# arghyasur1991/Spark-TTS

Measured on AMD Instinct MI355X. Metric: audio samples/sec (whole node), Spark-TTS-0.5B greedy, higher is better.
Workload: dtype bf16 weights + KV, fp32 activations/accumulate (LLM); vocoder: fp32 operands split into 2 bf16 planes, 3 products on the bf16 matrix pipe, fp32 accumulate

## Files before the change

include/sparkmi_debug.h:

```cpp
#ifndef SPARKMI_DEBUG_H
#define SPARKMI_DEBUG_H

#include "sparkmi.h"

#ifdef __cplusplus
extern "C" {
#endif

int smi_llm_time_kernel(smi_llm* h, int kernel, int layer, int iters, float* ms_avg, void* stream);
int smi_llm_debug_stamps(smi_llm* h, int kernel, int layer, double* out);
int smi_llm_engine(smi_llm* h, int32_t* enabled, int32_t* info, char* why, int n);
int smi_llm_set_engine(smi_llm* h, int on);
int smi_llm_engine_plan(const smi_llm_cfg* cfg, int ncu, int32_t* stats);
int smi_llm_engine_stamps(smi_llm* h, double* out, int cap);
int smi_llm_debug_hidden(smi_llm* h, float* out_host, int n);
int smi_llm_debug_read(smi_llm* h, int what, void* out_host, size_t cap, size_t* got);

int smi_llm_debug_set_kv(smi_llm* h, int layer, int slot, int pos0, int n, const float* k_host, const float* v_host);
int smi_llm_debug_get_kv(smi_llm* h, int layer, int slot, int pos0, int n, float* k_host, float* v_host);
int smi_llm_debug_layer(smi_llm* h, int layer, int M, const int32_t* rows_host, const float* hidden_host, int stage);
enum { SMI_PF_GROUPED = 1, SMI_PF_PGEMM = 2 };
int smi_llm_debug_prefill_layer(smi_llm* h, int layer, int stage, int n_seq, const int32_t* seq_host, const float* hidden_host, int family);
int smi_llm_pf_tiles(const int32_t* rows_host, int M, int32_t* out, int cap, int32_t* n);
int smi_llm_debug_raw_stamps(smi_llm* h, unsigned long long* out, int n);
int smi_llm_debug_sample(smi_llm* h, const float* logits_host, int n_rows, uint64_t seed, int use_bound, int32_t* tokens_out);
int smi_llm_debug_penalize(smi_llm* h, const float* logits_host, int n_rows, const uint16_t* hist_host, const smi_penalty_params* pens,
                           const int32_t* emitted_host, float* logits_out, int32_t* argmax_out);
int smi_llm_debug_logprob(smi_llm* h, const float* logits_host, int n_rows, const float* temperature_host, const int32_t* tokens_host,
                          float* lp_out);
// ... 66 lines not shown
```

spark-tts_amd/csrc/smi_llm.hip:

```cpp
#include "smi_common.h"
#include <stdio.h>
#include <string.h>
#include <atomic>
#include <cmath>
#include <cstddef>
#include <map>
#include <mutex>
#include <vector>

namespace {

constexpr int kMaxRows = SMI_MAX_ROWS;
constexpr int kHeadDim = 64;

struct RowDesc {
  int32_t slot, pos, token, flags;
};

struct SampRec {
  int32_t mode;
  int32_t top_k;
  float inv_temp, top_p;
  unsigned long long seed;
  int32_t has_seed, pad;
// ... 1576 lines not shown
      red[(wave * NTB + nb) * 64 + lane] = make_float4(t[0], t[1], t[2], t[3]);
    }
    __syncthreads();
    if (wave < NTB) {
      const int nb = wave, nt = RT ? (g * NTB + nb < ntl ? p.tlist[1 + g * NTB + nb] : NT) : g * NTB + nb;
      if (nt < NT) {
        float4 s = red[(0 * NTB + nb) * 64 + lane];
#pragma unroll
        for (int wv = 1; wv < NW; ++wv) {
          const float4 t = red[(wv * NTB + nb) * 64 + lane];
          s.x += t.x; s.y += t.y; s.z += t.z; s.w += t.w;
        }
        s.x *= rn; s.y *= rn; s.z *= rn; s.w *= rn;
        const int n = nt * 16 + 4 * (lane >> 4);
        const bool valid = em < M;
        if (RT && valid) lm_mask4(p.ctl, p.rows[m0 + em].slot, n, s);
        if (valid && p.Y) {
          float* y = p.Y + (size_t)(m0 + em) * p.V + n;
          if (n + 0 < p.V) y[0] = s.x;
          if (n + 1 < p.V) y[1] = s.y;
          if (n + 2 < p.V) y[2] = s.z;
          if (n + 3 < p.V) y[3] = s.w;
        }
        float bv = -INFINITY;
        int bi = 0x7fffffff;
        const float sv[4] = {s.x, s.y, s.z, s.w};
#pragma unroll
        for (int r = 0; r < 4; ++r)
          if (n + r < p.V && sv[r] > bv) { bv = sv[r]; bi = n + r; }
#pragma unroll
        for (int o = 16; o <= 32; o <<= 1) {
// ... 10 lines not shown
    }
    __syncthreads();
  }
  if (tid < M) {
    float bv = -INFINITY;
    int bi = 0x7fffffff;
#pragma unroll
    for (int nb = 0; nb < NTB; ++nb) {
      const float ov = bestv[nb * 32 + tid];
      const int oi = besti[nb * 32 + tid];
      if (ov > bv || (ov == bv && oi < bi)) { bv = ov; bi = oi; }
    }
    p.pval[(size_t)(m0 + tid) * gridDim.x + blockIdx.x] = bv;
    p.pidx[(size_t)(m0 + tid) * gridDim.x + blockIdx.x] = bi;
  }
}


template <int UW, int RT = 0>
__global__ __launch_bounds__(256) void k_lm32(GemmP p, int ngroups_arg, int m0) {
  constexpr int NTB = 2, NW = 4, U = UW;
  extern __shared__ __attribute__((aligned(16))) unsigned char smem[];
  const int tid = threadIdx.x, lane = tid & 63, wave = tid >> 6;
  const int KT = p.KT, NT = p.NT;
  const int ntl = RT ? p.tlist[0] : 0;
  const int ngroups = RT ? (ntl + NTB - 1) / NTB : ngroups_arg;
  const int M = p.M - m0 < 32 ? p.M - m0 : 32;
  float4* red = (float4*)smem;
  float* rarr = (float*)(smem + (size_t)NW * NTB * 2 * 1024);
  float* bestv = rarr + 32;
// ... 1644 lines not shown
  float* apart; size_t apart_floats;
  int slot_busy[kMaxRows], slot_len[kMaxRows];
  int slot_plen[kMaxRows];
  uint64_t handle_id, session_gen;
  std::vector<unsigned char> host_blob;
  int do_sample, top_k; float temperature, top_p; unsigned long long seed;
  uint8_t slot_feat[kMaxRows];
  int lm_restrict;
  int seq_dirty[kMaxRows];
  SeqRec* seq;
  std::vector<SeqRec> hseq;
  int32_t* pctx;
  std::vector<int32_t> host_pctx;
  int* tlist;
  std::vector<int32_t> host_tlist;
  float* lp;
  float* lp_part; float2* lp_rowc;
  uint16_t* phist;
  int64_t* poll_dev; int64_t* poll_host;
  int32_t* pen_idx; size_t pen_idx_cap;
  std::vector<int32_t> host_pen_idx;
  float* logits; int* tok;
  float* cand_v; int* cand_i; unsigned int* cand_n;
  unsigned long long* stamps; int stamps_on;
  int max_steps;
  int tune[4];
  int graph_steps;
  int pf_inline;
  int pf_qkv_eighths;
  int prefetch_mask, prefetch_rows;
// ... 546 lines not shown
      break;
  }
  return p;
}

AttnP attn_operands(const smi_llm* L, int layer, const Work& w, const RowDesc* rows, int M) {
  const smi_llm_cfg& c = L->cfg;
  AttnP a;
  memset(&a, 0, sizeof(a));
  a.q = w.q; a.kcache = kv_layer(L, L->kcache, layer); a.vcache = kv_layer(L, L->vcache, layer);
  a.rows = rows; a.xs_out = w.xs_attn; a.M = M; a.q_dim = L->Q; a.n_kv = c.num_kv_heads;
  a.group = c.num_heads / c.num_kv_heads; a.max_pos = c.max_positions; a.n_heads = c.num_heads; a.km = kv_map(L);
  return a;
}

int launch_one(smi_llm* L, int which, int layer, const RowDesc* rows, int M, float* logits, hipStream_t st) {
  const smi_llm_cfg& c = L->cfg;
  const bool fused = fuse_o_now(L, rows, M);
  GemmP p = gemm_operands(L, which, layer, L->dec, rows, M, L->NTh * 4);
  if (which == KLM) p.Y = logits ? logits : (logits_needed(L, step_feat(L)) ? L->logits : nullptr);
  if (L->exact) {
    switch (which) {
      case KQKV: return launch_gemm_x<PRO_NORM, EPI_QKV>(L, p, st);
      case KO: return launch_gemm_x<PRO_PLAIN, EPI_RESID>(L, p, st);
      case KGU: return launch_gemm_x<PRO_NORM, EPI_SWIGLU>(L, p, st);
      case KD: return launch_gemm_x<PRO_PLAIN, EPI_RESID>(L, p, st);
      case KLM:
        SMI_REQUIRE((L->NTlm + 3) / 4 <= L->lm_cap, "lm_head partial buffer too small");
        return launch_gemm_x<PRO_NORM, EPI_LM>(L, p, st);
    }
// ... 55 lines not shown
        return launch_down_chains(L, p, st);
      switch (L->tune[3]) {
        case 2: return launch_gemm<1, 16, 3, 4, PRO_PLAIN, EPI_RESID>(L, p, st);
        case 4: return launch_gemm<1, 8, 10, 2, PRO_PLAIN, EPI_RESID>(L, p, st);
        case 5: return launch_gemm<1, 16, 2, 5, PRO_PLAIN, EPI_RESID, 2>(L, p, st);
        case 6: return launch_gemm<1, 16, 2, 5, PRO_PLAIN, EPI_RESID>(L, p, st);
        default:
          if (M <= 8) return launch_gemm<1, 16, 2, 5, PRO_PLAIN, EPI_RESID, 4>(L, p, st);
          if (M <= 16) return launch_gemm<1, 16, 2, 5, PRO_PLAIN, EPI_RESID, 4, 0>(L, p, st);
          if (M <= 32) return launch_gemm<1, 16, 2, 5, PRO_PLAIN, EPI_RESID, 2, 0>(L, p, st);
          return launch_gemm<1, 16, 2, 5, PRO_PLAIN, EPI_RESID, 1, 0>(L, p, st);
      }
    case KLM: {
      const unsigned feat = step_feat(L);
      p.stamps = L->stamps_on ? L->stamps : nullptr;
      if (L->KTh <= 32 && !logits && rows == L->rows && lm_restricted(L, feat)) {
        p.tlist = L->tlist; p.ctl = L->ctl;
        const size_t lds = (size_t)4 * 2 * 1024 + 32 * 4 + 2 * 32 * 8;
        const size_t lds32 = (size_t)4 * 2 * 2 * 1024 + 32 * 4 + 2 * 32 * 8 + (size_t)L->KTh * 12 * 16 * 16;
        if (M <= 16) {
          hipLaunchKernelGGL((k_lm<1, 1>), dim3(L->lm_blocks), dim3(256), lds, st, p, 0, 0);
          SMI_LAUNCH_CHECK();
          return SMI_OK;
        }
        for (int m0 = 0; m0 < M; m0 += 32) {
          if (!(L->tune2 & 8192) && lds32 <= 150 * 1024) {
            if (L->KTh <= 28) hipLaunchKernelGGL((k_lm32<7, 1>), dim3(lm_blocks_for(L, M)), dim3(256), lds32, st, p, 0, m0);
            else hipLaunchKernelGGL((k_lm32<8, 1>), dim3(lm_blocks_for(L, M)), dim3(256), lds32, st, p, 0, m0);
          } else
            hipLaunchKernelGGL((k_lm<2, 1>), dim3(lm_blocks_for(L, M)), dim3(512), 2 * lds, st, p, 0, m0);
// ... 14 lines not shown
              if (L->KTh <= 28) hipLaunchKernelGGL(k_lm32<7>, dim3(lm_blocks_for(L, M)), dim3(256), lds32, st, p, ngroups, m0);
              else hipLaunchKernelGGL(k_lm32<8>, dim3(lm_blocks_for(L, M)), dim3(256), lds32, st, p, ngroups, m0);
            } else
              hipLaunchKernelGGL(k_lm<2>, dim3(lm_blocks_for(L, M)), dim3(512), 2 * lds, st, p, ngroups, m0);
            SMI_LAUNCH_CHECK();
          }
        }
        return SMI_OK;
      }
      SMI_REQUIRE((L->NTlm + 3) / 4 <= L->lm_cap, "lm_head partial buffer too small");
      return launch_gemm<4, 4, 2, 1, PRO_NORM, EPI_LM>(L, p, st);
    }
    case KFIN: {
      const unsigned feat = step_feat(L);
      FinP f = fin_params(L, M);
      if (feat & F_NGRAM) {
        size_t lds;
        const NgramP np = ngram_params(L, &lds);
        hipLaunchKernelGGL(k_ngram_ban, dim3(1, M), dim3(256), lds, st, np);
        SMI_LAUNCH_CHECK();
      }
      if ((feat & (F_PEN | F_BIAS | F_NGRAM)) || ((feat & F_ALLOW) && logits_needed(L, feat))) {
        PenP pp = pen_params(L, M);
        if (feat & F_BIAS) pp.seq = L->seq;
        hipLaunchKernelGGL(k_penalize, dim3((pp.nblk + kPenWaves - 1) / kPenWaves, M), dim3(256), 0, st, pp);
        SMI_LAUNCH_CHECK();
        f.phist = L->phist;
      }
      if (feat & F_SAMPLE) {
        const SampleP sp = sample_params(L, M);
// ... 407 lines not shown
    for (int i = 0; i < 4; ++i) { const char* e = smi_env(names[i]); L->pg_forced |= e != nullptr; L->pg_min[i] = e ? atoi(e) : common ? L->pgemm_min_rows : dflt[i]; }
  }
  { const char* e = smi_env("SPARKMI_PG_SPLIT_ROWS"); L->pg_split_rows = e ? atoi(e) : kPgSplitRows; if (L->pg_split_rows > kPgSplitRows) L->pg_split_rows = kPgSplitRows; }
  { const char* e = smi_env("SPARKMI_PF_LONG"); L->pf_long = e ? atoi(e) : kMaxRows + 1; if (L->pf_long < kMaxRows + 1) L->pf_long = kMaxRows + 1; }
  { const char* e = smi_env("SPARKMI_GU1_ROWS"); L->gu1_rows = e ? atoi(e) : 32; }
  { const char* e = smi_env("SPARKMI_GU1_LO"); L->gu1_lo = e ? atoi(e) : 4; }
  L->wd_parts = cfg->wd_plain ? 0 : 1;
  L->exact = cfg->weights_exact;
  if (L->exact) L->fuse_o = 0;
  L->pf_tiles = nullptr; L->pf_tiles_cap = 0; L->pf_ntiles = 0;
  L->dbg_pf_rows = 0;
  { const char* e = smi_env("SPARKMI_ATTN_PF2"); L->attn_pf2 = !(e && e[0] == '0'); }
  L->graph = nullptr; L->graph_id = 0; slots_clear(L);
  L->lp = nullptr; L->lp_part = nullptr; L->lp_rowc = nullptr;
  L->tlist = nullptr;
  memset(L->seq_dirty, 0, sizeof(L->seq_dirty));
  L->seq = nullptr; L->hseq.assign(kMaxRows, SeqRec{});
  L->pctx = nullptr;
  L->poll_dev = nullptr; L->poll_host = nullptr;
  L->phist = nullptr; L->pen_idx = nullptr; L->pen_idx_cap = 0; L->plan = nullptr; L->plan_cap = 0; L->B = 0; L->started = 0; L->ctl = nullptr; L->admit_seq = 0; memset(&L->hctl, 0, sizeof(L->hctl));
  L->session = 0; L->identity_slots = 1; L->attn_seg = 1; L->apart = nullptr; L->apart_floats = 0; memset(L->slot_busy, 0, sizeof(L->slot_busy)); memset(L->slot_len, 0, sizeof(L->slot_len));
  memset(L->slot_plen, 0, sizeof(L->slot_plen));
  { static std::atomic<uint64_t> handles{0}; L->handle_id = ++handles; L->session_gen = 0; }
  const size_t esz = cfg->kv_dtype ? 4 : 2;
  L->paged = cfg->kv_page_tokens > 0; L->pshift = 0; L->ppslot = 0; L->ptab = nullptr;
  memset(L->slot_pages, 0, sizeof(L->slot_pages));
  L->kv_layer_elems = (size_t)cfg->max_slots * cfg->num_kv_heads * cfg->max_positions * kHeadDim;
  if (L->paged) {
    while ((1 << L->pshift) < cfg->kv_page_tokens) ++L->pshift;
    L->ppslot = cfg->max_positions >> L->pshift;
// ... 83 lines not shown
    int dev = 0;
    std::lock_guard<std::mutex> lk(mu);
    if (hipGetDevice(&dev) != hipSuccess || dev < 0 || dev >= 64) {
      smi_set_error("smi_llm_create: no current device");
      smi_llm_destroy(L);
      return SMI_EHIP;
    }
    for (size_t i = 0; i < lds_big_kernels().size() && !done[dev]; ++i)
      if (hipFuncSetAttribute(lds_big_kernels()[i], hipFuncAttributeMaxDynamicSharedMemorySize, kLdsBigBytes) != hipSuccess) {
        smi_set_error("smi_llm_create: hipFuncSetAttribute(MaxDynamicSharedMemorySize) failed: %s", hipGetErrorString(hipGetLastError()));
        smi_llm_destroy(L);
        return SMI_EHIP;
      }
    done[dev] = true;
  }
  if (hipEventCreate(&L->ev0) != hipSuccess || hipEventCreate(&L->ev1) != hipSuccess) {
    smi_set_error("hipEventCreate failed");
    smi_llm_destroy(L);
    return SMI_EHIP;
  }
#ifdef SMI_DIAG
  L->eng_on = 0;
  snprintf(L->eng.why, sizeof(L->eng.why), "off (opt-in: SPARKMI_ENGINE=1 or smi_llm_set_engine)");
  { const char* e = smi_env("SPARKMI_ENGINE");
    if (e && e[0] == '1') {
      const int rce = eng_create(L);
      if (rce) { smi_llm_destroy(L); return rce; }
      L->eng_on = L->eng.enabled;
    }
  }
#endif
  *out = L;
  return SMI_OK;
}

int smi_llm_destroy(smi_llm* L) {
  if (!L) return SMI_OK;
  graphs_flush(L);
  eng_destroy(L);
  work_free(L->dec);
  work_free(L->big);
  void* ptrs[] = {L->part_o, L->h2, L->dpart, L->fuse_cnt, L->rows, L->plan, L->pf_tiles, L->pval, L->pidx, L->hist,
                  L->count, L->finished, L->step, L->ctl, L->ptab, L->kcache, L->vcache, L->logits, L->tok, L->cand_v, L->cand_i, L->cand_n, L->stamps, L->pslab, L->apart,
                  L->phist, L->pen_idx, L->lp, L->lp_part, L->lp_rowc, L->tlist, L->poll_dev, L->seq, L->pctx};
  for (void* q : ptrs)
    if (q) (void)hipFree(q);
  if (L->poll_host) (void)hipHostFree(L->poll_host);
  if (L->ev0) (void)hipEventDestroy(L->ev0);
  if (L->ev1) (void)hipEventDestroy(L->ev1);
  delete L;
  return SMI_OK;
}

int smi_llm_set_sampling(smi_llm* L, int do_sample, float temperature, int top_k, float top_p, uint64_t seed) {
  SMI_REQUIRE(L, "smi_llm_set_sampling: null handle");
  if (do_sample) {
    SMI_REQUIRE(temperature > 0.f, "smi_llm_set_sampling: temperature must be > 0");
    SMI_REQUIRE(top_k >= 1 && top_k <= kSampleCap, "smi_llm_set_sampling: top_k must be in 1..%d", kSampleCap);
    SMI_REQUIRE(top_p > 0.f && top_p <= 1.f, "smi_llm_set_sampling: top_p must be in (0, 1]");
// ... 1353 lines not shown

int smi_llm_set_engine(smi_llm* L, int on) {
  SMI_REQUIRE(L, "smi_llm_set_engine: null handle");
  int v = on ? 1 : 0;
  if (v && !L->eng.enabled) {
    SMI_HIP(hipDeviceSynchronize());
    const int rce = eng_create(L);
    if (rce) return rce;
    v = L->eng.enabled;
  }
  if (v != L->eng_on) { SMI_HIP(hipDeviceSynchronize()); graphs_flush(L); }
  L->eng_on = v;
  return SMI_OK;
}

int smi_llm_engine_plan(const smi_llm_cfg* cfg, int ncu, int32_t* stats) {
  SMI_REQUIRE(cfg_ok(cfg) && stats, "smi_llm_engine_plan: invalid argument");
  EngPlanHost P;
  char why[128] = "";
  const int Q = cfg->num_heads * cfg->head_dim, KV = cfg->num_kv_heads * cfg->head_dim;
  if (!eng_build_plan(cfg->hidden_size, Q, KV, cfg->intermediate_size, cfg->num_heads, ncu, P, why, sizeof(why))) {
    smi_set_error("engine plan: %s", why);
    return SMI_EINVAL;
  }
  long total = 0, want = 0;
  for (int ph = 0; ph < 4; ++ph) want += (long)P.g.nparts[ph] * P.g.part_imgs[ph];
  std::vector<unsigned char> seen[4];
  for (int ph = 0; ph < 4; ++ph) seen[ph].assign((size_t)P.g.nparts[ph] * 4 * 64, 0);
  for (int c = 0; c < ncu; ++c)
    for (int w = 0; w < kEngWaves; ++w) {
// ... 509 lines not shown
```

spark-tts_amd/sparkmi/_lib.py:

```python
from __future__ import annotations

import ctypes as C
import os
from pathlib import Path

_HERE = Path(__file__).resolve().parent
LIB_PATH = Path(os.environ["SPARKMI_LIB"]) if os.environ.get("SPARKMI_LIB") else _HERE / "libsparkmi.so"

SMI_MAX_ROWS = 64
SMI_MAX_EOS = 4
ABI_VERSION = 4


class SparkMIError(RuntimeError):
    pass


class LLMCfg(C.Structure):
    _fields_ = [(n, C.c_int32) for n in (
        "vocab_size", "hidden_size", "num_layers", "num_heads", "num_kv_heads", "head_dim",
        "intermediate_size", "max_slots", "max_positions", "kv_dtype", "use_graph")] + [("rms_eps", C.c_float),
                                                                                        ("kv_page_tokens", C.c_int32), ("kv_pages", C.c_int32), ("wd_plain", C.c_int32),
                                                                                        ("weights_exact", C.c_int32)]

# ... 154 lines not shown
    "smi_enc_arena_bytes": (_SZ, [_P(EncCfg)]),
    "smi_enc_create": (_I, [_P(EncCfg), _VP, _SZ, _P(_VP)]),
    "smi_enc_destroy": (_I, [_VP]),
    "smi_enc_forward": (_I, [_VP, _VP, _I, _VP, _I, _VP, _VP, _P(_I), _VP]),
    "smi_enc_debug_stage": (_I, [_VP, C.c_char_p, _VP, _SZ, _P(C.c_int32), _VP]),
    "smi_enc_num_launches": (_I, [_VP]),
    "smi_enc_time_launch": (_I, [_VP, _I, _I, _P(C.c_float), _P(C.c_double), C.c_char_p, _I, _VP]),
}

DEBUG_SYMBOLS = {
    "smi_llm_time_kernel": (_I, [_VP, _I, _I, _I, _P(C.c_float), _VP]),
    "smi_llm_debug_stamps": (_I, [_VP, _I, _I, _P(C.c_double)]),
    "smi_llm_engine": (_I, [_VP, _P(C.c_int32), _P(C.c_int32), C.c_char_p, _I]),
    "smi_llm_set_engine": (_I, [_VP, _I]),
    "smi_llm_engine_plan": (_I, [_P(LLMCfg), _I, _P(C.c_int32)]),
    "smi_llm_engine_stamps": (_I, [_VP, _P(C.c_double), _I]),
    "smi_llm_debug_hidden": (_I, [_VP, _P(C.c_float), _I]),
    "smi_llm_debug_read": (_I, [_VP, _I, _VP, _SZ, _P(_SZ)]),
    "smi_llm_debug_raw_stamps": (_I, [_VP, _P(C.c_uint64), _I]),
    "smi_llm_debug_sample": (_I, [_VP, _P(C.c_float), _I, C.c_uint64, _I, _P(C.c_int32)]),
    "smi_llm_debug_logprob": (_I, [_VP, _P(C.c_float), _I, _P(C.c_float), _P(C.c_int32), _P(C.c_float)]),
    "smi_llm_debug_penalize": (_I, [_VP, _P(C.c_float), _I, _P(C.c_uint16), _P(PenaltyParams), _P(C.c_int32), _P(C.c_float),
                                    _P(C.c_int32)]),
    "smi_llm_debug_seqbias": (_I, [_VP, _P(C.c_float), _I, _P(SeqParams), _P(C.c_int64), _P(C.c_int32), _P(C.c_int32), _I,
                                   _P(C.c_int32), _P(C.c_float), _P(C.c_int32), _P(C.c_int32)]),
    "smi_llm_debug_ngram": (_I, [_VP, _P(C.c_float), _I, _P(C.c_int32), _P(C.c_int64), _P(C.c_int32), _P(C.c_int32), _I,
                                 _P(C.c_float), _P(C.c_int32)]),
    "smi_llm_debug_set_kv": (_I, [_VP, _I, _I, _I, _I, _P(C.c_float), _P(C.c_float)]),
    "smi_llm_debug_get_kv": (_I, [_VP, _I, _I, _I, _I, _P(C.c_float), _P(C.c_float)]),
    "smi_llm_debug_layer": (_I, [_VP, _I, _I, _P(C.c_int32), _P(C.c_float), _I]),
# ... 75 lines not shown
```

spark-tts_amd/sparkmi/llm.py:

```python
from __future__ import annotations

import ctypes as C
import itertools
import json
import warnings
from pathlib import Path
from typing import Iterable, List, Mapping, Optional, Sequence, Union

import numpy as np
import torch

from . import _lib
from .arena import llm_cfg_struct, pack_llm_arena
from .config import LLMConfig


EosLike = Union[None, int, Iterable[int]]
SAMPLING_KEYS = ("do_sample", "temperature", "top_k", "top_p", "seed")
PENALTY_KEYS = ("repetition_penalty", "presence_penalty", "frequency_penalty", "min_new_tokens", "penalize_prompt")
PENALTY_NEUTRAL = dict(repetition_penalty=1.0, presence_penalty=0.0, frequency_penalty=0.0, min_new_tokens=0)
LOGPROB_KEYS = ("return_log_probs",)
ALLOW_KEY = "allowed_token_ids"


# ... 304 lines not shown
            host = pack_llm_arena(cfg, weights, self._cs)
            arena = torch.from_numpy(host).to(self.device)
        else:
            off, nb = C.c_size_t(), C.c_size_t()
            self._lib.check(self._lib.smi_llm_arena_section(C.byref(self._cs), _lib.LLM_TAG, 0, C.byref(off), C.byref(nb)),
                            "smi_llm_arena_section")
            if arena.numel() >= off.value + nb.value:
                tag = _lib.LLMArenaTag.from_buffer_copy(arena[off.value: off.value + nb.value].cpu().numpy().tobytes())
                if tag.magic == b"SMIARENA":
                    self._cs.wd_plain = tag.wd_plain
        self.arena = arena
        self._sampling = dict(do_sample=False, temperature=0.8, top_k=50, top_p=0.95)
        self._h = C.c_void_p()
        self._lib.check(self._lib.smi_llm_create(C.byref(self._cs), C.c_void_p(arena.data_ptr()),
                                            arena.numel(), C.byref(self._h)), "smi_llm_create")

    def _stream(self) -> C.c_void_p:
        return C.c_void_p(torch.cuda.current_stream(self.device).cuda_stream)

    def close(self) -> None:
        if getattr(self, "_h", None) is not None and self._h:
            self._lib.smi_llm_destroy(self._h)
            self._h = C.c_void_p()

    def __del__(self):
        try:
            self.close()
        except Exception:
            pass

# ... 388 lines not shown
                                    "diag=True (libsparkmi_diag.so); the product library does not export it")

    def engine_info(self) -> dict:
        self._need_diag("engine_info")
        on = C.c_int32(0)
        info = (C.c_int32 * 4)()
        why = C.create_string_buffer(200)
        self._lib.check(self._lib.smi_llm_engine(self._h, C.byref(on), info, why, 200), "smi_llm_engine")
        return {"enabled": bool(on.value), "built": bool(info[3]), "cus": int(info[0]), "images_per_wave": int(info[1]),
                "lds_bytes": int(info[2]), "why": why.value.decode(errors="replace")}

    def set_engine(self, on: bool) -> None:
        self._need_diag("set_engine")
        self._lib.check(self._lib.smi_llm_set_engine(self._h, 1 if on else 0), "smi_llm_set_engine")

    def engine_stamps(self) -> np.ndarray:
        self._need_diag("engine_stamps")
        n = 3 * self.cfg.num_hidden_layers * 16
        out = (C.c_double * n)()
        self._lib.check(self._lib.smi_llm_engine_stamps(self._h, out, n), "smi_llm_engine_stamps")
        return np.array(out, dtype=np.float64).reshape(3, self.cfg.num_hidden_layers, 16)

    def debug_hidden(self) -> np.ndarray:
        self._need_diag("debug_hidden")
        out = np.zeros(self.cfg.hidden_size, dtype=np.float32)
        self._lib.check(self._lib.smi_llm_debug_hidden(self._h, out.ctypes.data_as(C.POINTER(C.c_float)), out.size), "smi_llm_debug_hidden")
        return out

    def debug_read(self, what: int, nbytes: int = 1 << 22) -> np.ndarray:
        self._need_diag("debug_read")
# ... 175 lines not shown
        self._lib.check(self._lib.smi_llm_debug_logprob(self._h, lg.ctypes.data_as(C.POINTER(C.c_float)), n,
                                                        t.ctypes.data_as(C.POINTER(C.c_float)),
                                                        tk.ctypes.data_as(C.POINTER(C.c_int32)),
                                                        out.ctypes.data_as(C.POINTER(C.c_float))), "smi_llm_debug_logprob")
        return out

    KERNELS = ("qkv", "attn", "o_proj", "gate_up", "down", "lm_head", "finalize", "step", "layers")

    def time_kernel(self, name: str, iters: int = 48, layer: int = 0, in_sequence: bool = False) -> float:
        self._need_diag("time_kernel")
        ms = C.c_float(0)
        self._lib.check(self._lib.smi_llm_time_kernel(self._h, self.KERNELS.index(name) + (16 if in_sequence else 0), layer, iters,
                                                 C.byref(ms), self._stream()), "smi_llm_time_kernel")
        return float(ms.value)

    def weight_bytes(self) -> dict:
        c = self.cfg
        h, q, kv, i = c.hidden_size, c.q_dim, c.kv_dim, c.intermediate_size
        return {"qkv": 2 * (q + 2 * kv) * h, "o_proj": 2 * h * q, "gate_up": 2 * 2 * i * h, "down": 2 * h * i,
                "lm_head": 2 * c.vocab_size * h}

    def step_weight_bytes(self) -> int:
        w = self.weight_bytes()
        per_layer = w["qkv"] + w["o_proj"] + w["gate_up"] + w["down"]
        return self.cfg.num_hidden_layers * per_layer + w["lm_head"]

    def kv_bytes_per_token(self) -> int:
        esz = 4 if self._cs.kv_dtype else 2
        return self.cfg.num_hidden_layers * 2 * self.cfg.kv_dim * esz
```

Before: 563,900.

## Screen LM head with int8 bounds and compute exact logits only for candidate tiles

Builds an int8-quantized copy of the LM-head weights with per-row scale and error norms at engine creation. For greedy decoding with up to 16 rows, each step quantizes the hidden state, runs an int8 MFMA screen that produces rigorous upper and lower bounds per vocab tile, selects the tiles whose upper bound reaches the best lower bound, and runs the exact bf16 LM-head kernel only on those tiles. This halves the LM-head weight bytes read per step, at the cost of three extra kernel launches, extra device memory, and a correctness dependence on the error-bound derivation.

Result: slower. 556,100 (-1.4%).

```diff
diff --git a/include/sparkmi_debug.h b/include/sparkmi_debug.h
--- a/include/sparkmi_debug.h
+++ b/include/sparkmi_debug.h
@@ -13,6 +13,12 @@
 int smi_llm_set_engine(smi_llm* h, int on);
 int smi_llm_engine_plan(const smi_llm_cfg* cfg, int ncu, int32_t* stats);
 int smi_llm_engine_stamps(smi_llm* h, double* out, int cap);
+int smi_llm_set_lm_screen(smi_llm* h, int on);
+int smi_llm_lm_screen_info(smi_llm* h, int64_t* info);
+int smi_llm_lm_screen_copy(smi_llm* h, void* q_host, float* sen_host);
+int smi_llm_lm_screen_last(smi_llm* h, int n_rows, int32_t* cand, float* thr, int32_t* tiles_host);
+int smi_llm_debug_lm_screen(smi_llm* h, int M, const float* hidden_host, float* lo_host, float* up_host, float* logits_host,
+                            int32_t* tok_screen, int32_t* tok_full);
 int smi_llm_debug_hidden(smi_llm* h, float* out_host, int n);
 int smi_llm_debug_read(smi_llm* h, int what, void* out_host, size_t cap, size_t* got);
 
diff --git a/spark-tts_amd/csrc/smi_llm.hip b/spark-tts_amd/csrc/smi_llm.hip
--- a/spark-tts_amd/csrc/smi_llm.hip
+++ b/spark-tts_amd/csrc/smi_llm.hip
@@ -1614,7 +1614,7 @@
         s.x *= rn; s.y *= rn; s.z *= rn; s.w *= rn;
         const int n = nt * 16 + 4 * (lane >> 4);
         const bool valid = em < M;
-        if (RT && valid) lm_mask4(p.ctl, p.rows[m0 + em].slot, n, s);
+        if (RT == 1 && valid) lm_mask4(p.ctl, p.rows[m0 + em].slot, n, s);
         if (valid && p.Y) {
           float* y = p.Y + (size_t)(m0 + em) * p.V + n;
           if (n + 0 < p.V) y[0] = s.x;
@@ -1655,6 +1655,243 @@
     p.pval[(size_t)(m0 + tid) * gridDim.x + blockIdx.x] = bv;
     p.pidx[(size_t)(m0 + tid) * gridDim.x + blockIdx.x] = bi;
   }
+}
+
+typedef __attribute__((ext_vector_type(4))) int i32x4;
+constexpr int kScreenWaves = 4;
+constexpr int kScreenExact = 128;
+constexpr float kScreenUp = 1.001f;
+
+__global__ __launch_bounds__(256) void k_lmq_build(const uint4* __restrict__ W, int NT, int KT, int KQ, int V, uint4* __restrict__ Q,
+                                                    float* __restrict__ SEN) {
+  const int lane = threadIdx.x & 63, nt = blockIdx.x * 4 + ((int)threadIdx.x >> 6);
+  if (nt >= NT) return;
+  const int g = lane >> 4, n = lane & 15;
+  const bool row_ok = nt * 16 + n < V;
+  auto load16 = [&](int kq, float* w) {
+    const int kt = 2 * kq + (g >> 1);
+    const bool ok = row_ok && kt < KT;
+    const int ktc = kt < KT ? kt : KT - 1;
+#pragma unroll
+    for (int h = 0; h < 2; ++h) {
+      const uint4 v = W[((size_t)nt * KT + ktc) * 64 + (2 * (g & 1) + h) * 16 + n];
+      const uint32_t u[4] = {v.x, v.y, v.z, v.w};
+#pragma unroll
+      for (int i = 0; i < 4; ++i) {
+        w[h * 8 + 2 * i] = ok ? smi_bf16_to_f32(u[i] & 0xffffu) : 0.f;
+        w[h * 8 + 2 * i + 1] = ok ? smi_bf16_to_f32(u[i] >> 16) : 0.f;
+      }
+    }
+  };
+  float amax = 0.f;
+  for (int kq = 0; kq < KQ; ++kq) {
+    float w[16];
+    load16(kq, w);
+#pragma unroll
+    for (int i = 0; i < 16; ++i) amax = fmaxf(amax, fabsf(w[i]));
+  }
+  amax = fmaxf(amax, __shfl_xor(amax, 16, 64));
+  amax = fmaxf(amax, __shfl_xor(amax, 32, 64));
+  const float S = __fdiv_rn(amax, 127.0f);
+  float e2 = 0.f, n2 = 0.f;
+  for (int kq = 0; kq < KQ; ++kq) {
+    float w[16];
+    load16(kq, w);
+    uint32_t pk[4] = {0u, 0u, 0u, 0u};
+#pragma unroll
+    for (int i = 0; i < 16; ++i) {
+      float qf = S > 0.f ? rintf(__fdiv_rn(w[i], S)) : 0.f;
+      qf = fminf(fmaxf(qf, -127.f), 127.f);
+      const float d = fmaf(-S, qf, w[i]), r = S * qf;
+      e2 += d * d;
+      n2 += r * r;
+      pk[i >> 2] |= ((uint32_t)(int)qf & 0xffu) << (8 * (i & 3));
+    }
+    Q[((size_t)nt * KQ + kq) * 64 + lane] = make_uint4(pk[0], pk[1], pk[2], pk[3]);
+  }
+  e2 += __shfl_xor(e2, 16, 64); e2 += __shfl_xor(e2, 32, 64);
+  n2 += __shfl_xor(n2, 16, 64); n2 += __shfl_xor(n2, 32, 64);
+  if (g == 0) {
+    SEN[((size_t)nt * 3 + 0) * 16 + n] = S;
+    SEN[((size_t)nt * 3 + 1) * 16 + n] = sqrtf(e2) * kScreenUp;
+    SEN[((size_t)nt * 3 + 2) * 16 + n] = sqrtf(n2) * kScreenUp;
+  }
+}
+
+struct ScreenP {
+  const uint4* Q;
+  const float* SEN;
+  const unsigned char* XS;
+  const float* sspart; int npart; float eps;
+  int M, KT, KQ, NT, V;
+  uint4* xq;
+  float4* xsc;
+  float* ub;
+  float* lb;
+  int nwaves;
+  int* tl;
+  float* dbg;
+};
+
+__global__ __launch_bounds__(256) void k_lm_xq(ScreenP p) {
+  __shared__ float s_red[2][4];
+  const int m = blockIdx.x, tid = threadIdx.x, lane = tid & 63, wave = tid >> 6;
+  const int K = p.KT * 32, k0 = tid * 4;
+  float x[4] = {0.f, 0.f, 0.f, 0.f};
+  if (k0 < K) {
+    uint2 t[3];
+#pragma unroll
+    for (int s = 0; s < 3; ++s) t[s] = *(const uint2*)(p.XS + xs_off(k0 >> 5, s, (k0 >> 3) & 3, m, p.M) + (k0 & 7) * 2);
+    const uint32_t hi[2] = {t[0].x, t[0].y}, mi[2] = {t[1].x, t[1].y}, lo[2] = {t[2].x, t[2].y};
+#pragma unroll
+    for (int i = 0; i < 2; ++i) {
+      x[2 * i] = (smi_bf16_to_f32(hi[i] & 0xffffu) + smi_bf16_to_f32(mi[i] & 0xffffu)) + smi_bf16_to_f32(lo[i] & 0xffffu);
+      x[2 * i + 1] = (smi_bf16_to_f32(hi[i] >> 16) + smi_bf16_to_f32(mi[i] >> 16)) + smi_bf16_to_f32(lo[i] >> 16);
+    }
+  }
+  float amax = fmaxf(fmaxf(fabsf(x[0]), fabsf(x[1])), fmaxf(fabsf(x[2]), fabsf(x[3])));
+  float ss = (x[0] * x[0] + x[1] * x[1]) + (x[2] * x[2] + x[3] * x[3]);
+#pragma unroll
+  for (int o = 1; o < 64; o <<= 1) amax = fmaxf(amax, __shfl_xor(amax, o, 64));
+  ss = smi_wave_sum(ss);
+  if (lane == 0) { s_red[0][wave] = amax; s_red[1][wave] = ss; }
+  __syncthreads();
+  amax = fmaxf(fmaxf(s_red[0][0], s_red[0][1]), fmaxf(s_red[0][2], s_red[0][3]));
+  ss = (s_red[1][0] + s_red[1][1]) + (s_red[1][2] + s_red[1][3]);
+  const float c = amax > 1e-30f ? __fdiv_rn(16256.0f, amax) : 0.f;
+  if (k0 < p.KQ * 64) {
+    uint32_t q1 = 0u, q2 = 0u;
+#pragma unroll
+    for (int i = 0; i < 4; ++i) {
+      int T = (int)rintf(x[i] * c);
+      T = T > 16256 ? 16256 : (T < -16256 ? -16256 : T);
+      const int a = (T + 64) >> 7, b = T - 128 * a;
+      q1 |= ((uint32_t)a & 0xffu) << (8 * i);
+      q2 |= ((uint32_t)b & 0xffu) << (8 * i);
+    }
+    const size_t o = ((size_t)(k0 >> 6) * 2 * 64 + ((k0 >> 4) & 3) * 16 + m) * 16 + (k0 & 15);
+    *(uint32_t*)((unsigned char*)p.xq + o) = q1;
+    *(uint32_t*)((unsigned char*)p.xq + o + 64 * 16) = q2;
+  }
+  if (wave == 0) {
+    float v = smi_ss_lane_sum(p.sspart + (size_t)m * p.npart, p.npart, lane);
+    v = smi_wave_sum(v);
+    if (lane == 0) {
+      const float rn = 1.0f / sqrtf(v / (float)(p.KT * 32) + p.eps);
+      const float X = sqrtf(ss) * kScreenUp;
+      const float sqK = sqrtf((float)(p.KQ * 64)) * kScreenUp;
+      const float ex = (c > 0.f ? __fdiv_rn(0.501f, c) : amax) * sqK * kScreenUp + X * 0x1p-22f;
+      const float gam = (float)(p.KT * 32) * 0x1p-23f;
+      const float infl = 1.0f + 0x1p-18f;
+      p.xsc[m] = make_float4(c > 0.f ? __fdiv_rn(rn, c) : 0.f, rn * (X + gam * X) * infl, rn * (ex + gam * X) * infl, 0.f);
+    }
+  }
+}
+
+template <int KQC>
+__global__ __launch_bounds__(64 * kScreenWaves) void k_lm_screen(ScreenP p) {
+  const int lane = threadIdx.x & 63, wave = (int)threadIdx.x >> 6;
+  const int wg = blockIdx.x * kScreenWaves + wave, nw = gridDim.x * kScreenWaves;
+  const int KQ = p.KQ, NT = p.NT, M = p.M;
+  const int g = lane >> 4, em = lane & 15;
+  i32x4 wA[KQC], wB[KQC];
+  float4 cA[3], cB[3];
+  auto req = [&](int t, i32x4* w, float4* c) {
+    t = t < NT ? t : NT - 1;
+#pragma unroll
+    for (int u = 0; u < KQC; ++u) {
+      const int j = u < KQ ? u : KQ - 1;
+      w[u] = __builtin_bit_cast(i32x4, smi_ldw(&p.Q[((size_t)t * KQ + j) * 64 + lane]));
+    }
+#pragma unroll
+    for (int s = 0; s < 3; ++s) c[s] = *(const float4*)(p.SEN + ((size_t)t * 3 + s) * 16 + 4 * g);
+  };
+  req(wg, wA, cA);
+  req(wg + nw, wB, cB);
+  asm volatile("" ::: "memory");
+  i32x4 x1[KQC], x2[KQC];
+#pragma unroll
+  for (int u = 0; u < KQC; ++u) {
+    const int j = u < KQ ? u : KQ;
+    x1[u] = __builtin_bit_cast(i32x4, p.xq[((size_t)j * 2 + 0) * 64 + lane]);
+    x2[u] = __builtin_bit_cast(i32x4, p.xq[((size_t)j * 2 + 1) * 64 + lane]);
+  }
+  const float4 sc = p.xsc[em < M ? em : 0];
+  float lrun = -INFINITY;
+  auto tile = [&](int t, const i32x4* w, const float4* c) {
+    i32x4 a1 = {0, 0, 0, 0}, a2 = {0, 0, 0, 0};
+#pragma unroll
+    for (int u = 0; u < KQC; ++u) {
+      a1 = __builtin_amdgcn_mfma_i32_16x16x64_i8(w[u], x1[u], a1, 0, 0, 0);
+      a2 = __builtin_amdgcn_mfma_i32_16x16x64_i8(w[u], x2[u], a2, 0, 0, 0);
+    }
+    const float S[4] = {c[0].x, c[0].y, c[0].z, c[0].w}, E[4] = {c[1].x, c[1].y, c[1].z, c[1].w}, N[4] = {c[2].x, c[2].y, c[2].z, c[2].w};
+    const int n = t * 16 + 4 * g;
+    float up = -INFINITY, lo = -INFINITY;
+#pragma unroll
+    for (int i = 0; i < 4; ++i) {
+      const float s = ((float)a1[i] * 128.0f + (float)a2[i]) * (S[i] * sc.x);
+      const float b = ((E[i] * sc.y + N[i] * sc.z) + fabsf(s) * 0x1p-21f) * (1.0f + 0x1p-20f);
+      if (n + i < p.V) { up = fmaxf(up, s + b); lo = fmaxf(lo, s - b); }
+      if (p.dbg && n + i < p.V && em < M) {
+        p.dbg[(size_t)em * NT * 16 + n + i] = s - b;
+        p.dbg[(size_t)(16 + em) * NT * 16 + n + i] = s + b;
+      }
+    }
+    up = fmaxf(up, __shfl_xor(up, 16, 64)); up = fmaxf(up, __shfl_xor(up, 32, 64));
+    lo = fmaxf(lo, __shfl_xor(lo, 16, 64)); lo = fmaxf(lo, __shfl_xor(lo, 32, 64));
+    if (lane < 16) p.ub[(size_t)t * 16 + lane] = up;
+    lrun = fmaxf(lrun, lo);
+  };
+  for (int t = wg; t < NT; t += 2 * nw) {
+    tile(t, wA, cA);
+    req(t + 2 * nw, wA, cA);
+    if (t + nw < NT) tile(t + nw, wB, cB);
+    req(t + 3 * nw, wB, cB);
+  }
+  if (lane < 16 && wg < p.nwaves) p.lb[(size_t)wg * 16 + lane] = lrun;
+}
+
+__global__ __launch_bounds__(1024) void k_lm_select(ScreenP p) {
+  __shared__ float s_l[64][16];
+  __shared__ float s_L[16];
+  __shared__ int s_cnt[16];
+  const int tid = threadIdx.x, lane = tid & 63, wave = tid >> 6;
+  {
+    const int m = tid & 15;
+    float l = -INFINITY;
+    for (int w = tid >> 4; w < p.nwaves; w += 64) l = fmaxf(l, p.lb[(size_t)w * 16 + m]);
+    s_l[tid >> 4][m] = l;
+  }
+  __syncthreads();
+  if (tid < 16) {
+    float l = -INFINITY;
+    for (int i = 0; i < 64; ++i) l = fmaxf(l, s_l[i][tid]);
+    s_L[tid] = l;
+  }
+  __syncthreads();
+  const int per = (p.NT + 1023) / 1024, t0 = tid * per, t1 = t0 + per < p.NT ? t0 + per : p.NT;
+  auto is_cand = [&](int t) {
+    bool f = false;
+    for (int m = 0; m < p.M; ++m) f |= p.ub[(size_t)t * 16 + m] >= s_L[m];
+    return f;
+  };
+  int cnt = 0;
+  for (int t = t0; t < t1; ++t) cnt += is_cand(t) ? 1 : 0;
+  int inc = cnt;
+#pragma unroll
+  for (int o = 1; o < 64; o <<= 1) {
+    const int v = __shfl_up(inc, o, 64);
+    if (lane >= o) inc += v;
+  }
+  if (lane == 63) s_cnt[wave] = inc;
+  __syncthreads();
+  int base = 0, total = 0;
+  for (int w = 0; w < 16; ++w) { if (w < wave) base += s_cnt[w]; total += s_cnt[w]; }
+  int o = base + inc - cnt;
+  for (int t = t0; t < t1; ++t)
+    if (is_cand(t) && o < p.NT) p.tl[1 + o++] = t;
+  if (tid == 0) p.tl[0] = total < p.NT ? total : p.NT;
 }
 
 
@@ -3329,6 +3566,8 @@
   std::vector<int32_t> host_pctx;
   int* tlist;
   std::vector<int32_t> host_tlist;
+  uint4* lmq; float* lm_sen; uint4* sc_xq; float4* sc_xsc; float* sc_ub; float* sc_lb; int* sc_tl;
+  int lm_kq, sc_blocks, lm_screen; size_t lmq_bytes;
   float* lp;
   float* lp_part; float2* lp_rowc;
   uint16_t* phist;
@@ -3905,6 +4144,66 @@
   return a;
 }
 
+bool lm_screen_now(const smi_llm* L, int M, unsigned feat) {
+  return L->lmq && L->lm_screen && M >= 1 && M <= 16 && feat == 0;
+}
+int lm_screen_exact_blocks(const smi_llm* L) { return L->lm_blocks < kScreenExact ? L->lm_blocks : kScreenExact; }
+
+int lm_screen_create(smi_llm* L) {
+  if (L->exact || L->KTh > 32) return SMI_OK;
+  int ncu = 0;
+  { int dev = 0; if (hipGetDevice(&dev) != hipSuccess || hipDeviceGetAttribute(&ncu, hipDeviceAttributeMultiprocessorCount, dev) != hipSuccess) ncu = 0; }
+  L->sc_blocks = ncu >= 1 && ncu <= 1024 ? ncu : 256;
+  L->lm_kq = (L->KTh + 1) / 2;
+  const size_t NT = (size_t)L->NTlm, qb = NT * L->lm_kq * 1024, sb = NT * 3 * 16 * 4;
+  const size_t xb = ((size_t)L->lm_kq + 1) * 2 * 1024, ub = NT * 16 * 4, lb = (size_t)L->sc_blocks * kScreenWaves * 16 * 4, tb = (NT + 1) * 4;
+  if (hipMalloc((void**)&L->lmq, qb) != hipSuccess || hipMalloc((void**)&L->lm_sen, sb) != hipSuccess ||
+      hipMalloc((void**)&L->sc_xq, xb) != hipSuccess || hipMalloc((void**)&L->sc_xsc, 16 * sizeof(float4)) != hipSuccess ||
+      hipMalloc((void**)&L->sc_ub, ub) != hipSuccess || hipMalloc((void**)&L->sc_lb, lb) != hipSuccess ||
+      hipMalloc((void**)&L->sc_tl, tb) != hipSuccess) {
+    (void)hipGetLastError();
+    void* ptrs[] = {L->lmq, L->lm_sen, L->sc_xq, L->sc_xsc, L->sc_ub, L->sc_lb, L->sc_tl};
+    for (void* q : ptrs) if (q) (void)hipFree(q);
+    L->lmq = nullptr; L->lm_sen = nullptr; L->sc_xq = nullptr; L->sc_xsc = nullptr; L->sc_ub = nullptr; L->sc_lb = nullptr; L->sc_tl = nullptr;
+    return SMI_OK;
+  }
+  L->lmq_bytes = qb + sb + xb + 16 * sizeof(float4) + ub + lb + tb;
+  SMI_HIP(hipMemset(L->sc_xq, 0, xb));
+  SMI_HIP(hipMemset(L->sc_xsc, 0, 16 * sizeof(float4)));
+  SMI_HIP(hipMemset(L->sc_ub, 0, ub));
+  SMI_HIP(hipMemset(L->sc_lb, 0, lb));
+  SMI_HIP(hipMemset(L->sc_tl, 0, tb));
+  hipLaunchKernelGGL(k_lmq_build, dim3((unsigned)((NT + 3) / 4)), dim3(256), 0, 0, (const uint4*)sec(L, SMI_LLM_LM_HEAD, 0), L->NTlm, L->KTh,
+                     L->lm_kq, L->cfg.vocab_size, L->lmq, L->lm_sen);
+  SMI_LAUNCH_CHECK();
+  SMI_HIP(hipDeviceSynchronize());
+  L->lm_screen = 1;
+  return SMI_OK;
+}
+
+int launch_lm_screen(smi_llm* L, GemmP p, int M, hipStream_t st, float* dbg) {
+  ScreenP s;
+  memset(&s, 0, sizeof(s));
+  s.Q = L->lmq; s.SEN = L->lm_sen; s.XS = p.XS; s.sspart = p.sspart; s.npart = p.npart; s.eps = p.eps;
+  s.M = M; s.KT = p.KT; s.KQ = L->lm_kq; s.NT = p.NT; s.V = p.V;
+  s.xq = L->sc_xq; s.xsc = L->sc_xsc; s.ub = L->sc_ub; s.lb = L->sc_lb; s.nwaves = L->sc_blocks * kScreenWaves; s.tl = L->sc_tl; s.dbg = dbg;
+  hipLaunchKernelGGL(k_lm_xq, dim3(M), dim3(256), 0, st, s);
+  SMI_LAUNCH_CHECK();
+  const dim3 grid(L->sc_blocks), block(64 * kScreenWaves);
+  if (s.KQ <= 4) hipLaunchKernelGGL(k_lm_screen<4>, grid, block, 0, st, s);
+  else if (s.KQ <= 8) hipLaunchKernelGGL(k_lm_screen<8>, grid, block, 0, st, s);
+  else if (s.KQ <= 14) hipLaunchKernelGGL(k_lm_screen<14>, grid, block, 0, st, s);
+  else hipLaunchKernelGGL(k_lm_screen<16>, grid, block, 0, st, s);
+  SMI_LAUNCH_CHECK();
+  hipLaunchKernelGGL(k_lm_select, dim3(1), dim3(1024), 0, st, s);
+  SMI_LAUNCH_CHECK();
+  p.tlist = L->sc_tl; p.Y = nullptr;
+  const size_t lds = (size_t)4 * 2 * 1024 + 32 * 4 + 2 * 32 * 8;
+  hipLaunchKernelGGL((k_lm<1, 2>), dim3(lm_screen_exact_blocks(L)), dim3(256), lds, st, p, 0, 0);
+  SMI_LAUNCH_CHECK();
+  return SMI_OK;
+}
+
 int launch_one(smi_llm* L, int which, int layer, const RowDesc* rows, int M, float* logits, hipStream_t st) {
   const smi_llm_cfg& c = L->cfg;
   const bool fused = fuse_o_now(L, rows, M);
@@ -3990,6 +4289,7 @@
     case KLM: {
       const unsigned feat = step_feat(L);
       p.stamps = L->stamps_on ? L->stamps : nullptr;
+      if (!logits && rows == L->rows && lm_screen_now(L, M, feat)) return launch_lm_screen(L, p, M, st, nullptr);
       if (L->KTh <= 32 && !logits && rows == L->rows && lm_restricted(L, feat)) {
         p.tlist = L->tlist; p.ctl = L->ctl;
         const size_t lds = (size_t)4 * 2 * 1024 + 32 * 4 + 2 * 32 * 8;
@@ -4034,6 +4334,7 @@
     case KFIN: {
       const unsigned feat = step_feat(L);
       FinP f = fin_params(L, M);
+      if (lm_screen_now(L, M, feat)) f.nblk = lm_screen_exact_blocks(L);
       if (feat & F_NGRAM) {
         size_t lds;
         const NgramP np = ngram_params(L, &lds);
@@ -4471,6 +4772,8 @@
   L->graph = nullptr; L->graph_id = 0; slots_clear(L);
   L->lp = nullptr; L->lp_part = nullptr; L->lp_rowc = nullptr;
   L->tlist = nullptr;
+  L->lmq = nullptr; L->lm_sen = nullptr; L->sc_xq = nullptr; L->sc_xsc = nullptr; L->sc_ub = nullptr; L->sc_lb = nullptr; L->sc_tl = nullptr;
+  L->lm_kq = 0; L->sc_blocks = 0; L->lm_screen = 0; L->lmq_bytes = 0;
   memset(L->seq_dirty, 0, sizeof(L->seq_dirty));
   L->seq = nullptr; L->hseq.assign(kMaxRows, SeqRec{});
   L->pctx = nullptr;
@@ -4584,6 +4887,7 @@
       }
     done[dev] = true;
   }
+  { const int rcs = lm_screen_create(L); if (rcs) { smi_llm_destroy(L); return rcs; } }
   if (hipEventCreate(&L->ev0) != hipSuccess || hipEventCreate(&L->ev1) != hipSuccess) {
     smi_set_error("hipEventCreate failed");
     smi_llm_destroy(L);
@@ -4612,7 +4916,8 @@
   work_free(L->big);
   void* ptrs[] = {L->part_o, L->h2, L->dpart, L->fuse_cnt, L->rows, L->plan, L->pf_tiles, L->pval, L->pidx, L->hist,
                   L->count, L->finished, L->step, L->ctl, L->ptab, L->kcache, L->vcache, L->logits, L->tok, L->cand_v, L->cand_i, L->cand_n, L->stamps, L->pslab, L->apart,
-                  L->phist, L->pen_idx, L->lp, L->lp_part, L->lp_rowc, L->tlist, L->poll_dev, L->seq, L->pctx};
+                  L->phist, L->pen_idx, L->lp, L->lp_part, L->lp_rowc, L->tlist, L->poll_dev, L->seq, L->pctx,
+                  L->lmq, L->lm_sen, L->sc_xq, L->sc_xsc, L->sc_ub, L->sc_lb, L->sc_tl};
   for (void* q : ptrs)
     if (q) (void)hipFree(q);
   if (L->poll_host) (void)hipHostFree(L->poll_host);
@@ -5996,6 +6301,113 @@
   return SMI_OK;
 }
 
+int smi_llm_set_lm_screen(smi_llm* L, int on) {
+  SMI_REQUIRE(L, "smi_llm_set_lm_screen: null handle");
+  const int v = on && L->lmq ? 1 : 0;
+  if (v != L->lm_screen) { SMI_HIP(hipDeviceSynchronize()); graphs_flush(L); }
+  L->lm_screen = v;
+  return SMI_OK;
+}
+
+int smi_llm_lm_screen_info(smi_llm* L, int64_t* info) {
+  SMI_REQUIRE(L && info, "smi_llm_lm_screen_info: null argument");
+  info[0] = L->lmq ? 1 : 0; info[1] = L->lm_screen; info[2] = L->lm_kq; info[3] = L->NTlm; info[4] = L->sc_blocks;
+  info[5] = lm_screen_exact_blocks(L); info[6] = (int64_t)L->lmq_bytes; info[7] = (int64_t)L->NTlm * L->lm_kq * 1024;
+  return SMI_OK;
+}
+
+int smi_llm_lm_screen_copy(smi_llm* L, void* q_host, float* sen_host) {
+  SMI_REQUIRE(L && q_host && sen_host, "smi_llm_lm_screen_copy: null argument");
+  SMI_REQUIRE(L->lmq, "smi_llm_lm_screen_copy: this engine has no int8 copy (exact weights, or hidden size beyond 1024)");
+  SMI_HIP(hipDeviceSynchronize());
+  SMI_HIP(hipMemcpy(q_host, L->lmq, (size_t)L->NTlm * L->lm_kq * 1024, hipMemcpyDeviceToHost));
+  SMI_HIP(hipMemcpy(sen_host, L->lm_sen, (size_t)L->NTlm * 3 * 16 * 4, hipMemcpyDeviceToHost));
+  return SMI_OK;
+}
+
+int smi_llm_lm_screen_last(smi_llm* L, int n_rows, int32_t* cand, float* thr, int32_t* tiles_host) {
+  SMI_REQUIRE(L && cand && thr && n_rows >= 1 && n_rows <= 16, "smi_llm_lm_screen_last: bad argument");
+  SMI_REQUIRE(L->lmq, "smi_llm_lm_screen_last: this engine has no int8 copy");
+  SMI_HIP(hipDeviceSynchronize());
+  const size_t NT = (size_t)L->NTlm, nw = (size_t)L->sc_blocks * kScreenWaves;
+  std::vector<float> ub(NT * 16), lb(nw * 16);
+  SMI_HIP(hipMemcpy(ub.data(), L->sc_ub, ub.size() * 4, hipMemcpyDeviceToHost));
+  SMI_HIP(hipMemcpy(lb.data(), L->sc_lb, lb.size() * 4, hipMemcpyDeviceToHost));
+  for (int m = 0; m < n_rows; ++m) {
+    float l = -INFINITY;
+    for (size_t w = 0; w < nw; ++w) l = lb[w * 16 + m] > l ? lb[w * 16 + m] : l;
+    int c = 0;
+    for (size_t t = 0; t < NT; ++t) c += ub[t * 16 + m] >= l ? 1 : 0;
+    thr[m] = l; cand[m] = c;
+  }
+  if (tiles_host) SMI_HIP(hipMemcpy(tiles_host, L->sc_tl, (NT + 1) * 4, hipMemcpyDeviceToHost));
+  return SMI_OK;
+}
+
+static void lm_pick(const std::vector<float>& pv, const std::vector<int>& pi, int M, int nblk, int V, int32_t* tok) {
+  for (int m = 0; m < M; ++m) {
+    float bv = -INFINITY; int bi = 0x7fffffff;
+    for (int j = 0; j < nblk; ++j) {
+      const float v = pv[(size_t)m * nblk + j]; const int ix = pi[(size_t)m * nblk + j];
+      if (v > bv || (v == bv && ix < bi)) { bv = v; bi = ix; }
+    }
+    tok[m] = (unsigned)bi >= (unsigned)V ? 0 : bi;
+  }
+}
+int smi_llm_debug_lm_screen(smi_llm* L, int M, const float* hidden_host, float* lo_host, float* up_host, float* logits_host,
+                            int32_t* tok_screen, int32_t* tok_full) {
+  SMI_REQUIRE(L && hidden_host && lo_host && up_host && logits_host && tok_screen && tok_full && M >= 1 && M <= 16, "smi_llm_debug_lm_screen: bad argument");
+  SMI_REQUIRE(L->lmq, "smi_llm_debug_lm_screen: this engine has no int8 copy");
+  SMI_HIP(hipDeviceSynchronize());
+  graphs_flush(L);
+  std::vector<RowDesc> rows(kMaxRows, RowDesc{0, 0, 0, 0});
+  for (int m = 0; m < M; ++m) rows[m] = RowDesc{m, 0, 0, 0};
+  SMI_HIP(hipMemcpy(L->rows, rows.data(), rows.size() * sizeof(RowDesc), hipMemcpyHostToDevice));
+  L->B = M; L->identity_slots = 1; L->session = 0; L->started = 0; L->attn_seg = 1;
+  const int V = L->cfg.vocab_size;
+  const size_t NT16 = (size_t)L->NTlm * 16;
+  float *src = nullptr, *dbg = nullptr;
+  SMI_HIP(hipMalloc((void**)&src, (size_t)M * L->H * 4));
+  if (hipMalloc((void**)&dbg, 2 * 16 * NT16 * 4) != hipSuccess) { (void)hipFree(src); smi_set_error("smi_llm_debug_lm_screen: hipMalloc failed"); return SMI_ENOMEM; }
+  int rc = SMI_OK;
+  std::vector<float> pv; std::vector<int> pi;
+  auto run = [&]() -> int {
+    SMI_HIP(hipMemcpy(src, hidden_host, (size_t)M * L->H * 4, hipMemcpyHostToDevice));
+    SMI_HIP(hipMemset(dbg, 0, 2 * 16 * NT16 * 4));
+    hipLaunchKernelGGL(k_load_hidden, dim3((M + 3) / 4), dim3(256), 0, 0, src, L->KTh, M, (const float*)sec(L, SMI_LLM_FINAL_NORM, 0), L->dec.h,
+                       L->dec.xs_h, L->dec.ss, L->NTh * 4);
+    SMI_LAUNCH_CHECK();
+    GemmP p = gemm_operands(L, KLM, 0, L->dec, L->rows, M, L->NTh * 4);
+    int r = launch_lm_screen(L, p, M, 0, dbg);
+    if (r) return r;
+    SMI_HIP(hipDeviceSynchronize());
+    int nblk = lm_screen_exact_blocks(L);
+    pv.resize((size_t)M * nblk); pi.resize((size_t)M * nblk);
+    SMI_HIP(hipMemcpy(pv.data(), L->pval, pv.size() * 4, hipMemcpyDeviceToHost));
+    SMI_HIP(hipMemcpy(pi.data(), L->pidx, pi.size() * 4, hipMemcpyDeviceToHost));
+    lm_pick(pv, pi, M, nblk, V, tok_screen);
+    for (int m = 0; m < M; ++m) {
+      SMI_HIP(hipMemcpy(lo_host + (size_t)m * V, dbg + (size_t)m * NT16, (size_t)V * 4, hipMemcpyDeviceToHost));
+      SMI_HIP(hipMemcpy(up_host + (size_t)m * V, dbg + (size_t)(16 + m) * NT16, (size_t)V * 4, hipMemcpyDeviceToHost));
+    }
+    p.Y = L->logits;
+    const size_t lds = (size_t)4 * 2 * 1024 + 32 * 4 + 2 * 32 * 8;
+    hipLaunchKernelGGL(k_lm<1>, dim3(L->lm_blocks), dim3(256), lds, 0, p, (L->NTlm + 1) / 2, 0);
+    SMI_LAUNCH_CHECK();
+    SMI_HIP(hipDeviceSynchronize());
+    nblk = L->lm_blocks;
+    pv.resize((size_t)M * nblk); pi.resize((size_t)M * nblk);
+    SMI_HIP(hipMemcpy(pv.data(), L->pval, pv.size() * 4, hipMemcpyDeviceToHost));
+    SMI_HIP(hipMemcpy(pi.data(), L->pidx, pi.size() * 4, hipMemcpyDeviceToHost));
+    lm_pick(pv, pi, M, nblk, V, tok_full);
+    SMI_HIP(hipMemcpy(logits_host, L->logits, (size_t)M * V * 4, hipMemcpyDeviceToHost));
+    return SMI_OK;
+  };
+  rc = run();
+  (void)hipFree(src); (void)hipFree(dbg);
+  return rc;
+}
+
 int smi_llm_engine_plan(const smi_llm_cfg* cfg, int ncu, int32_t* stats) {
   SMI_REQUIRE(cfg_ok(cfg) && stats, "smi_llm_engine_plan: invalid argument");
   EngPlanHost P;
diff --git a/spark-tts_amd/sparkmi/_lib.py b/spark-tts_amd/sparkmi/_lib.py
--- a/spark-tts_amd/sparkmi/_lib.py
+++ b/spark-tts_amd/sparkmi/_lib.py
@@ -192,6 +192,12 @@
     "smi_llm_engine": (_I, [_VP, _P(C.c_int32), _P(C.c_int32), C.c_char_p, _I]),
     "smi_llm_set_engine": (_I, [_VP, _I]),
     "smi_llm_engine_plan": (_I, [_P(LLMCfg), _I, _P(C.c_int32)]),
+    "smi_llm_set_lm_screen": (_I, [_VP, _I]),
+    "smi_llm_lm_screen_info": (_I, [_VP, _P(C.c_int64)]),
+    "smi_llm_lm_screen_copy": (_I, [_VP, _VP, _P(C.c_float)]),
+    "smi_llm_lm_screen_last": (_I, [_VP, _I, _P(C.c_int32), _P(C.c_float), _P(C.c_int32)]),
+    "smi_llm_debug_lm_screen": (_I, [_VP, _I, _P(C.c_float), _P(C.c_float), _P(C.c_float), _P(C.c_float), _P(C.c_int32),
+                                     _P(C.c_int32)]),
     "smi_llm_engine_stamps": (_I, [_VP, _P(C.c_double), _I]),
     "smi_llm_debug_hidden": (_I, [_VP, _P(C.c_float), _I]),
     "smi_llm_debug_read": (_I, [_VP, _I, _VP, _SZ, _P(_SZ)]),
diff --git a/spark-tts_amd/sparkmi/llm.py b/spark-tts_amd/sparkmi/llm.py
--- a/spark-tts_amd/sparkmi/llm.py
+++ b/spark-tts_amd/sparkmi/llm.py
@@ -342,6 +342,7 @@
         self._h = C.c_void_p()
         self._lib.check(self._lib.smi_llm_create(C.byref(self._cs), C.c_void_p(arena.data_ptr()),
                                             arena.numel(), C.byref(self._h)), "smi_llm_create")
+        self._lm_screen = not weights_exact and cfg.hidden_size <= 1024
 
     def _stream(self) -> C.c_void_p:
         return C.c_void_p(torch.cuda.current_stream(self.device).cuda_stream)
@@ -760,6 +761,51 @@
         self._need_diag("set_engine")
         self._lib.check(self._lib.smi_llm_set_engine(self._h, 1 if on else 0), "smi_llm_set_engine")
 
+    def set_lm_screen(self, on: bool) -> None:
+        self._need_diag("set_lm_screen")
+        self._lib.check(self._lib.smi_llm_set_lm_screen(self._h, 1 if on else 0), "smi_llm_set_lm_screen")
+        self._lm_screen = bool(on) and self.lm_screen_info()["exists"]
+
+    def lm_screen_info(self) -> dict:
+        self._need_diag("lm_screen_info")
+        info = (C.c_int64 * 8)()
+        self._lib.check(self._lib.smi_llm_lm_screen_info(self._h, info), "smi_llm_lm_screen_info")
+        keys = ("exists", "on", "k_tiles", "tiles", "screen_blocks", "exact_blocks", "device_bytes", "q_bytes")
+        d = {k: int(v) for k, v in zip(keys, info)}
+        d["exists"], d["on"] = bool(d["exists"]), bool(d["on"])
+        return d
+
+    def lm_screen_copy(self):
+        i = self.lm_screen_info()
+        q = np.zeros((i["tiles"], i["k_tiles"], 64, 16), dtype=np.int8)
+        sen = np.zeros((i["tiles"], 3, 16), dtype=np.float32)
+        self._lib.check(self._lib.smi_llm_lm_screen_copy(self._h, q.ctypes.data_as(C.c_void_p), sen.ctypes.data_as(C.POINTER(C.c_float))),
+                        "smi_llm_lm_screen_copy")
+        return q, sen
+
+    def lm_screen_last(self, n_rows: int):
+        i = self.lm_screen_info()
+        cand = np.zeros(n_rows, dtype=np.int32)
+        thr = np.zeros(n_rows, dtype=np.float32)
+        tl = np.zeros(i["tiles"] + 1, dtype=np.int32)
+        ip = C.POINTER(C.c_int32)
+        self._lib.check(self._lib.smi_llm_lm_screen_last(self._h, n_rows, cand.ctypes.data_as(ip), thr.ctypes.data_as(C.POINTER(C.c_float)),
+                                                         tl.ctypes.data_as(ip)), "smi_llm_lm_screen_last")
+        return cand, thr, tl[1:1 + int(tl[0])].copy()
+
+    def debug_lm_screen(self, hidden: np.ndarray):
+        self._need_diag("debug_lm_screen")
+        hidden = np.ascontiguousarray(hidden, dtype=np.float32)
+        M, V = hidden.shape[0], self.cfg.vocab_size
+        assert hidden.shape == (M, self.cfg.hidden_size)
+        lo, up, lg = (np.zeros((M, V), dtype=np.float32) for _ in range(3))
+        ts, tf = np.zeros(M, dtype=np.int32), np.zeros(M, dtype=np.int32)
+        fp, ip = C.POINTER(C.c_float), C.POINTER(C.c_int32)
+        self._lib.check(self._lib.smi_llm_debug_lm_screen(self._h, M, hidden.ctypes.data_as(fp), lo.ctypes.data_as(fp), up.ctypes.data_as(fp),
+                                                          lg.ctypes.data_as(fp), ts.ctypes.data_as(ip), tf.ctypes.data_as(ip)),
+                        "smi_llm_debug_lm_screen")
+        return lo, up, lg, ts, tf
+
     def engine_stamps(self) -> np.ndarray:
         self._need_diag("engine_stamps")
         n = 3 * self.cfg.num_hidden_layers * 16
@@ -965,14 +1011,20 @@
                                                  C.byref(ms), self._stream()), "smi_llm_time_kernel")
         return float(ms.value)
 
-    def weight_bytes(self) -> dict:
+    def weight_bytes(self, rows: Optional[int] = None, greedy: Optional[bool] = None) -> dict:
         c = self.cfg
         h, q, kv, i = c.hidden_size, c.q_dim, c.kv_dim, c.intermediate_size
+        lm = 2 * c.vocab_size * h
+        rows = getattr(self, "_B", 1) if rows is None else rows
+        greedy = not self._sampling["do_sample"] if greedy is None else greedy
+        if self._lm_screen and greedy and rows <= 16:
+            vpad = (c.vocab_size + 15) // 16 * 16
+            lm = vpad * ((h + 63) // 64 * 64) + 12 * vpad
         return {"qkv": 2 * (q + 2 * kv) * h, "o_proj": 2 * h * q, "gate_up": 2 * 2 * i * h, "down": 2 * h * i,
-                "lm_head": 2 * c.vocab_size * h}
-
-    def step_weight_bytes(self) -> int:
-        w = self.weight_bytes()
+                "lm_head": lm}
+
+    def step_weight_bytes(self, rows: Optional[int] = None, greedy: Optional[bool] = None) -> int:
+        w = self.weight_bytes(rows, greedy)
         per_layer = w["qkv"] + w["o_proj"] + w["gate_up"] + w["down"]
         return self.cfg.num_hidden_layers * per_layer + w["lm_head"]
 
```
